# vkit-x/vkit

Measured on AMD Instinct MI355X. Metric: Mpixels/s (2048^2 RGB, geo+photo chain), higher is better.
Workload: dtype u8

## Files before the change

vkit_amd/csrc/nprand.hip:

```cpp
#include "vkx_internal.h"
#include "np_ziggurat.h"

#include <string.h>
#include <algorithm>

namespace {

typedef unsigned __int128 u128;
#define VKX_GLOBAL __attribute__((address_space(1)))

#ifndef VKX_NP_ROUNDS
#define VKX_NP_ROUNDS 48
#endif
constexpr int kRounds = VKX_NP_ROUNDS;
static_assert(kRounds % 2 == 0 && kRounds >= 2 && kRounds <= 64, "rounds per tile");
constexpr int kTile = 64 * kRounds;
constexpr double kNorR = 3.6541528853610087963519472518;
constexpr double kNorInvR = 0.27366123732975827203338247596;

#define PCG_MULT ((((u128)0x2360ED051FC65DA4ull) << 64) | (u128)0x4385DF649FCCF645ull)

struct JumpTabs {
    uint64_t pow2[64][4];
    uint64_t lane[64][4];
    uint64_t a64[2], g64[2];
    uint64_t a128[2], g128[2];
};
static JumpTabs g_jump_host;
static bool g_jump_host_ready = false;

static void jump_consts(u128 j, u128 *a, u128 *g)
{
    u128 acc_mult = 1, acc_plus = 0, cur_mult = PCG_MULT, cur_plus = 1;
    while (j > 0) {
        if (j & 1) {
            acc_mult *= cur_mult;
            acc_plus = acc_plus * cur_mult + cur_plus;
        }
        cur_plus = (cur_mult + 1) * cur_plus;
        cur_mult *= cur_mult;
        j >>= 1;
    }
    *a = acc_mult;
    *g = acc_plus;
}

static void build_jump_tabs()
{
    if (g_jump_host_ready) return;
    auto put = [](uint64_t *w, u128 a, u128 g) {
        w[0] = (uint64_t)a; w[1] = (uint64_t)(a >> 64); w[2] = (uint64_t)g; w[3] = (uint64_t)(g >> 64);
    };
    u128 a, g;
    for (int i = 0; i < 64; i++) { jump_consts((u128)1 << i, &a, &g); put(g_jump_host.pow2[i], a, g); }
    for (int l = 0; l < 64; l++) { jump_consts((u128)(l + 1), &a, &g); put(g_jump_host.lane[l], a, g); }
    jump_consts(64, &a, &g);
    g_jump_host.a64[0] = (uint64_t)a; g_jump_host.a64[1] = (uint64_t)(a >> 64);
    g_jump_host.g64[0] = (uint64_t)g; g_jump_host.g64[1] = (uint64_t)(g >> 64);
    jump_consts(128, &a, &g);
    g_jump_host.a128[0] = (uint64_t)a; g_jump_host.a128[1] = (uint64_t)(a >> 64);
    g_jump_host.g128[0] = (uint64_t)g; g_jump_host.g128[1] = (uint64_t)(g >> 64);
    g_jump_host_ready = true;
}

struct NpTabs {
    JumpTabs jump;
    uint64_t ki[256], wi[256], fi[256];
};

struct NpJob {
    uint64_t state[2], inc[2];
    uint64_t c64[2];
    uint64_t c128[2];
    long long n;
    long long tile_base;
    int n_tiles;
    int kind, cn;
    double loc, scale;
    double margin;
    double cdf[3];
    const uint8_t *src;
    void *dst;
    int16_t *rec;
    uint2 *table;
};

struct TileInfo {
    uint32_t count0, out0;
    uint64_t start0, emit0;
};
constexpr uint32_t kIrregular = 0x80000000u;
struct TilePlan {
    unsigned long long prefix;
    uint32_t c_in, count;
};

__device__ __forceinline__ u128 mk128(const uint64_t *w) { return ((u128)w[1] << 64) | (u128)w[0]; }

__device__ __forceinline__ uint64_t pcg_out(u128 s)
{
    const uint64_t hi = (uint64_t)(s >> 64), lo = (uint64_t)s;
    const uint64_t x = hi ^ lo;
    const unsigned r = (unsigned)(hi >> 58);
    return (x >> r) | (x << ((64 - r) & 63));
}
struct LcgStride {
    uint32_t a0, a1, a2, a3;
    uint64_t c0, c1, c23;
};
__device__ __forceinline__ LcgStride lcg_stride(u128 a, u128 c)
{
    LcgStride k;
    k.a0 = (uint32_t)a; k.a1 = (uint32_t)(a >> 32); k.a2 = (uint32_t)(a >> 64); k.a3 = (uint32_t)(a >> 96);
    k.c0 = (uint32_t)c; k.c1 = (uint32_t)(c >> 32); k.c23 = (uint64_t)(c >> 64);
    return k;
}
__device__ __forceinline__ uint64_t mad_u64_u32_v(uint32_t a, uint32_t b, uint64_t c)
{
    uint64_t d, carry;
    asm("v_mad_u64_u32 %0, %1, %2, %3, %4" : "=v"(d), "=s"(carry) : "v"(a), "v"(b), "v"(c));
    return d;
}
__device__ __forceinline__ uint64_t mul_u64_u32_v(uint32_t a, uint32_t b)
{
    uint64_t d, carry;
    asm("v_mad_u64_u32 %0, %1, %2, %3, 0" : "=v"(d), "=s"(carry) : "v"(a), "v"(b));
    return d;
}
__device__ __forceinline__ u128 lcg_step(u128 s, const LcgStride &k)
{
    const uint32_t s0 = (uint32_t)s, s1 = (uint32_t)(s >> 32), s2 = (uint32_t)(s >> 64), s3 = (uint32_t)(s >> 96);
    const uint64_t E = (uint64_t)k.a0 * s0 + k.c0;
    const uint64_t O1 = (uint64_t)k.a0 * s1 + k.c1;
    const uint64_t O2 = (uint64_t)k.a1 * s0;
    uint64_t F = (uint64_t)k.a0 * s2 + k.c23;
    F += (uint64_t)k.a1 * s1;
    F += (uint64_t)k.a2 * s0;
    uint64_t G = mul_u64_u32_v(k.a0, s3);
    G = mad_u64_u32_v(k.a1, s2, G);
    G = mad_u64_u32_v(k.a2, s1, G);
    G = mad_u64_u32_v(k.a3, s0, G);
    unsigned ca, cb, cc, cd;
    const uint32_t t = __builtin_addc((uint32_t)(E >> 32), (uint32_t)O1, 0u, &ca);
    const uint32_t r1 = __builtin_addc(t, (uint32_t)O2, 0u, &cb);
    const uint32_t u = __builtin_addc((uint32_t)F, (uint32_t)(O1 >> 32), ca, &cc);
    const uint32_t r2 = __builtin_addc(u, (uint32_t)(O2 >> 32), cb, &cd);
    unsigned ce;
    const uint32_t w = __builtin_addc((uint32_t)(F >> 32), (uint32_t)G, cc, &ce);
    const uint32_t r3 = __builtin_addc(w, 0u, cd, &ce);
    return ((u128)r3 << 96) | ((u128)r2 << 64) | ((u128)r1 << 32) | (uint32_t)E;
}

__device__ __forceinline__ double u2dbl(uint64_t u) { return (double)(long long)(u >> 11) * (1.0 / 9007199254740992.0); }

__device__ __forceinline__ int rounded_step(const NpJob &job, double z, bool inexact, uint32_t &flags)
{
    const double v = job.scale * z;
    if (inexact) {
        const double f = v - floor(v);
        if (fabs(f - 0.5) < 1e-9) flags |= VKX_NP_AMBIGUOUS;
    }
    return (int16_t)(int)__double_as_longlong(v + 6755399441055744.0);
}
struct EmitNone {
    typedef int Val;
    typedef int16_t Store;
    __device__ static Val make(const NpJob &, double, bool, uint32_t &) { return 0; }
    __device__ static void store(const NpJob &, void *, long long, Val, bool, uint32_t &) {}
};
struct EmitI16 {
    static constexpr bool kCheckAtStore = false;
    typedef int Val;
    typedef int16_t Store;
    __device__ static Val make(const NpJob &job, double z, bool inexact, uint32_t &flags) { return rounded_step(job, z, inexact, flags); }
    __device__ static void store(const NpJob &, void *dst, long long pos, Val k, bool, uint32_t &) { ((int16_t VKX_GLOBAL *)dst)[pos] = (int16_t)k; }
};
struct EmitAddU8 {
    static constexpr bool kCheckAtStore = false;
    typedef int Val;
    typedef int16_t Store;
    __device__ static Val make(const NpJob &job, double z, bool inexact, uint32_t &flags) { return rounded_step(job, z, inexact, flags); }
    __device__ static void store(const NpJob &job, void *dst, long long pos, Val k, bool, uint32_t &)
    {
        const int s = (int16_t)((int)((const uint8_t VKX_GLOBAL *)job.src)[pos] + k);
        ((uint8_t VKX_GLOBAL *)dst)[pos] = (uint8_t)vkd::clamp_u8(s);
    }
};
struct EmitSpeckle {
    static constexpr bool kCheckAtStore = true;
    typedef double Val;
    typedef double Store;
    __device__ static Val make(const NpJob &, double z, bool, uint32_t &) { return z; }
    __device__ static void store(const NpJob &job, void *dst, long long pos, Val z, bool inexact, uint32_t &flags)
    {
        const double noise = 0.0 + job.scale * z;
        const double m = (double)((const uint8_t VKX_GLOBAL *)job.src)[pos];
        const double t = m * noise;
        double r = m + t;
        if (inexact && m != 0.0 && fabs(r - rint(r)) < 1e-9) flags |= VKX_NP_AMBIGUOUS;
        r = r < 0.0 ? 0.0 : (r > 255.0 ? 255.0 : r);
        ((uint8_t VKX_GLOBAL *)dst)[pos] = (uint8_t)(int)r;
    }
};

constexpr int kEvCap = kRounds <= 48 ? 96 : 128;
template <typename Val, bool WITH_VAL>
struct WaveWork {
    uint64_t ev_s[kEvCap][2];
    uint16_t ev_pos[kEvCap];
    uint16_t ev_info[kEvCap];
    uint64_t slow[kRounds];
    uint64_t semit[kRounds];
    uint64_t cov[kRounds];
    __attribute__((aligned(16))) Val val[WITH_VAL ? kRounds : 1][64];
};

__device__ __forceinline__ uint64_t rfl64(uint64_t v)
{
    return ((uint64_t)(uint32_t)__builtin_amdgcn_readfirstlane((int)(v >> 32)) << 32) | (uint32_t)__builtin_amdgcn_readfirstlane((int)v);
}
__device__ __forceinline__ int mbcnt64(uint64_t m)
{
    return __builtin_amdgcn_mbcnt_hi((uint32_t)(m >> 32), __builtin_amdgcn_mbcnt_lo((uint32_t)m, 0u));
}

enum { kCount = 0, kRecord = 1, kEmit = 2, kCompact = 3 };

__device__ __forceinline__ uint32_t lds_offset(const void *p)
{
    return (uint32_t)(uintptr_t)(__attribute__((address_space(3))) const void *)p;
}

__device__ __forceinline__ uint32_t compact_tile_lds(int16_t *flat, uint64_t m)
{
    const uint32_t lane = (uint32_t)__lane_id();
    const uint32_t base = lds_offset(flat);
    uint32_t run = 0;
    constexpr int kBatch = 8;
    static_assert(kRounds % kBatch == 0 || kRounds < kBatch, "rounds per compaction batch");
#pragma unroll
    for (int r0 = 0; r0 < kRounds; r0 += kBatch) {
        uint32_t v[kBatch];
#pragma unroll
        for (int j = 0; j < kBatch; j++)
            if (r0 + j < kRounds) v[j] = (uint16_t)flat[64 * (r0 + j) + lane];
#pragma unroll
        for (int j = 0; j < kBatch; j++) {
            const int r = r0 + j;
            if (r >= kRounds) break;
            const uint32_t lo = (uint32_t)__builtin_amdgcn_readlane((int)m, r), hi = (uint32_t)__builtin_amdgcn_readlane((int)(m >> 32), r);
            const uint32_t rank = (uint32_t)__builtin_amdgcn_mbcnt_hi(hi, __builtin_amdgcn_mbcnt_lo(lo, run));
            const uint32_t addr = base + 2 * rank;
            const uint64_t mask = ((uint64_t)hi << 32) | lo;
            uint64_t saved;
            asm volatile("s_mov_b64 %[sv], exec\n\ts_mov_b64 exec, %[m]\n\tds_write_b16 %[a], %[v]\n\ts_mov_b64 exec, %[sv]"
                         : [sv] "=&s"(saved) : [m] "s"(mask), [a] "v"(addr), [v] "v"(v[j]) : "memory");
            run += (uint32_t)__builtin_popcountll(mask);
        }
    }
    __builtin_amdgcn_wave_barrier();
    return run;
}

template <class Emit, int MODE>
__device__ void walk_tile(const NpJob &job, const JumpTabs &g_jump, const uint4 *__restrict__ zig , const double *__restrict__ fi ,
                          WaveWork<typename Emit::Store, MODE == kEmit || MODE == kCompact> &ws, u128 base, uint32_t c_in, long long prefix,
                          long long draw_base, typename Emit::Store VKX_GLOBAL *rec_val, uint64_t VKX_GLOBAL *rec_mask, void *emit_dst,
                          uint32_t &count_out, uint32_t &carry_out, uint64_t &start0, uint64_t &emit0, bool &has_tail, uint32_t &flags,
                          unsigned long long *draws_used)
{
    const int lane = __lane_id();
    const u128 inc = mk128(job.inc);
    const u128 a64 = mk128(g_jump.a64), c64 = mk128(job.c64);
    c_in = (uint32_t)__builtin_amdgcn_readfirstlane((int)c_in);
    prefix = (long long)rfl64((uint64_t)prefix);
    draw_base = (long long)rfl64((uint64_t)draw_base);
    u128 s = mk128(&g_jump.lane[lane][0]) * base + mk128(&g_jump.lane[lane][2]) * inc;
    uint32_t nev = 0;
    if (lane < kRounds) ws.semit[lane] = 0;
    auto round = [&](int r, const u128 &st) {
        const uint64_t u = pcg_out(st);
        const int idx = (int)(u & 0xff);
        const uint64_t rabs = (u >> 9) & 0x000fffffffffffffull;
        const uint4 e = zig[idx];
        const uint64_t ki = ((uint64_t)e.y << 32) | e.x;
        if (MODE != kCount) {
            const double wi = __longlong_as_double(((long long)e.w << 32) | e.z);
            double x = (__longlong_as_double((long long)(0x4330000000000000ull | rabs)) - 4503599627370496.0) * wi;
            x = __longlong_as_double(__double_as_longlong(x) | ((long long)((uint32_t)u << 23 & 0x80000000u) << 32));
            const typename Emit::Store v = (typename Emit::Store)Emit::make(job, x, false, flags);
            if (MODE == kRecord) rec_val[64 * r + lane] = v;
            else if (MODE == kEmit || MODE == kCompact) ws.val[r][lane] = v;
        }
        const uint64_t slow = __ballot(rabs >= ki);
        if (lane == 0) ws.slow[r] = slow;
        if (slow) {
            if (rabs >= ki) {
                const uint32_t slot = nev + (uint32_t)mbcnt64(slow);
                if (slot < (uint32_t)kEvCap) {
                    ws.ev_s[slot][0] = (uint64_t)st;
                    ws.ev_s[slot][1] = (uint64_t)(st >> 64);
                    ws.ev_pos[slot] = (uint16_t)(64 * r + lane);
                }
            }
            nev += (uint32_t)__builtin_popcountll(slow);
        }
    };
    const LcgStride stride128 = lcg_stride(mk128(g_jump.a128), mk128(job.c128));
    u128 s2 = a64 * s + c64;
#pragma unroll 1
    for (int r = 0; r < kRounds; r += 2) {
        round(r, s);
        round(r + 1, s2);
        s = lcg_step(s, stride128);
        s2 = lcg_step(s2, stride128);
    }
    if (nev > (uint32_t)kEvCap) {
        flags |= VKX_NP_SHORT;
        nev = kEvCap;
    }
    __builtin_amdgcn_wave_barrier();
    if (MODE == kRecord) asm volatile("s_waitcnt vmcnt(0)" ::: "memory");
    has_tail = false;
#pragma unroll
    for (int q = 0; q < (kEvCap + 63) / 64; q++) {
        if ((uint32_t)(64 * q) >= nev) break;
        const uint32_t ev = 64 * q + lane;
        if (ev < nev) {
            const u128 se = ((u128)ws.ev_s[ev][1] << 64) | ws.ev_s[ev][0];
            const int pos = ws.ev_pos[ev];
            const uint64_t u = pcg_out(se);
            const int idx = (int)(u & 0xff);
            const uint64_t rabs = (u >> 9) & 0x000fffffffffffffull;
            uint32_t info;
            if (idx != 0) {
                double x = (__longlong_as_double((long long)(0x4330000000000000ull | rabs)) - 4503599627370496.0) *
                           __longlong_as_double(((long long)zig[idx].w << 32) | zig[idx].z);
                if (u & 0x100) x = -x;
                const double un = u2dbl(pcg_out(PCG_MULT * se + inc));
                const double f1 = fi[idx], f0 = fi[idx - 1];
                const double lhs = (f0 - f1) * un + f1;
                const double t = -0.5 * x;
                const double y = t * x;
                const float r32 = __builtin_amdgcn_exp2f((float)y * 1.44269504f);
                const float l32 = (float)lhs;
                bool accept = l32 < r32;
                if (fabsf(l32 - r32) <= r32 * 0x1p-14f || job.margin >= 1.0) {
                    const double rhs = exp(y);
                    if (fabs(rhs - lhs) <= lhs * job.margin) flags |= VKX_NP_AMBIGUOUS;
                    accept = lhs < rhs;
                }
                info = 2u | (accept ? 0x100u : 0u);
            } else {
                u128 t = se;
                uint32_t len = 1;
                double xx;
                for (;;) {
                    t = PCG_MULT * t + inc;
                    const double u1 = u2dbl(pcg_out(t));
                    t = PCG_MULT * t + inc;
                    const double u2 = u2dbl(pcg_out(t));
                    len += 2;
                    xx = -kNorInvR * log1p(-u1);
                    const double yy = -log1p(-u2);
                    const double l2 = yy + yy, r2 = xx * xx;
                    if (fabs(l2 - r2) <= r2 * 0x1p-40) flags |= VKX_NP_AMBIGUOUS;
                    if (l2 > r2 || len > 200) break;
                }
                if (len > 200) flags |= VKX_NP_SHORT;
                const double z = ((rabs >> 8) & 1) ? -(kNorR + xx) : kNorR + xx;
                if (MODE == kRecord) {
                    rec_val[pos] = (typename Emit::Store)Emit::make(job, z, true, flags);
                } else if (MODE == kCompact) {
                    (&ws.val[0][0])[pos] = (typename Emit::Store)Emit::make(job, z, true, flags);
                } else if (MODE == kEmit) {
                    const typename Emit::Val v = Emit::make(job, z, true, flags);
                    uint64_t bits = 0;
                    memcpy(&bits, &v, sizeof v);
                    ws.ev_s[ev][0] = bits;
                }
                has_tail = true;
                info = len | 0x300u;
            }
            ws.ev_info[ev] = (uint16_t)info;
            if (info & 0x100u) atomicOr((unsigned long long *)&ws.semit[pos >> 6], 1ull << (pos & 63));
        }
    }
    __builtin_amdgcn_wave_barrier();
    has_tail = __ballot(has_tail) != 0;
    uint32_t P = 0xffffu, end = 0, info = 0;
    if ((uint32_t)lane < nev) {
        P = ws.ev_pos[lane];
        info = ws.ev_info[lane];
        end = P + (info & 0xffu);
    }
    uint64_t valid;
    uint32_t carry = c_in > (uint32_t)kTile ? c_in - kTile : 0u;
    if (nev <= 64) {
        const uint32_t prev_end = (uint32_t)__builtin_amdgcn_update_dpp((int)c_in, (int)end, 0x138 , 0xf, 0xf, false);
        const uint64_t live = nev == 64 ? ~0ull : ((1ull << nev) - 1);
        const uint64_t touch = __ballot((uint32_t)lane < nev && P < prev_end);
        valid = live;
        if (touch) {
            uint32_t cover_end = c_in;
            valid = 0;
            for (uint32_t e = 0; e < nev; e++) {
                const uint32_t pe = (uint32_t)__builtin_amdgcn_readlane((int)P, (int)e);
                if (pe >= cover_end) {
                    valid |= 1ull << e;
                    cover_end = (uint32_t)__builtin_amdgcn_readlane((int)end, (int)e);
                }
            }
        }
        if (valid) {
            const uint32_t last_end = (uint32_t)__builtin_amdgcn_readlane((int)end, 63 - __builtin_clzll(valid));
            if (last_end > (uint32_t)kTile && last_end - kTile > carry) carry = last_end - kTile;
        }
        if (lane < kRounds) ws.cov[lane] = 0;
        __builtin_amdgcn_wave_barrier();
        if ((valid >> lane) & 1) {
            uint32_t p0 = P + 1, p1 = end < (uint32_t)kTile ? end : (uint32_t)kTile;
            while (p0 < p1) {
                const uint32_t r = p0 >> 6, stop = (r + 1) << 6 < p1 ? (r + 1) << 6 : p1;
                const uint32_t lo = p0 & 63, n = stop - p0;
                const uint64_t bits = (n == 64 ? ~0ull : ((1ull << n) - 1)) << lo;
                atomicOr((unsigned long long *)&ws.cov[r], bits);
                p0 = stop;
            }
        }
        __builtin_amdgcn_wave_barrier();
    } else {
        valid = 0;
        if (lane < kRounds) ws.cov[lane] = 0;
        __builtin_amdgcn_wave_barrier();
        uint32_t cover_end = c_in;
        for (uint32_t e = 0; e < nev; e++) {
            const uint32_t pe = ws.ev_pos[e], ee = pe + (ws.ev_info[e] & 0xffu);
            if (pe < cover_end) continue;
            cover_end = ee;
            if (lane == 0)
                for (uint32_t q = pe + 1; q < ee && q < (uint32_t)kTile; q++) ws.cov[q >> 6] |= 1ull << (q & 63);
        }
        if (cover_end > (uint32_t)kTile && cover_end - kTile > carry) carry = cover_end - kTile;
        __builtin_amdgcn_wave_barrier();
    }
    uint64_t my_mask = 0, my_starts = 0;
    if (lane < kRounds) {
        uint64_t cov = ws.cov[lane];
        const uint32_t lo = 64u * lane;
        if (c_in > lo) cov |= c_in - lo >= 64 ? ~0ull : ((1ull << (c_in - lo)) - 1);
        const uint64_t slow = ws.slow[lane];
        my_starts = ~cov;
        my_mask = my_starts & (~slow | ws.semit[lane]);
    }
    start0 = rfl64(my_starts);
    emit0 = rfl64(my_mask);
    uint32_t count = (uint32_t)__builtin_popcountll(my_mask);
    count += (uint32_t)__builtin_amdgcn_update_dpp(0, (int)count, 0x118 , 0xf, 0xf, true);
    count += (uint32_t)__builtin_amdgcn_update_dpp(0, (int)count, 0x114 , 0xf, 0xf, true);
    count += (uint32_t)__builtin_amdgcn_update_dpp(0, (int)count, 0x112 , 0xf, 0xf, true);
    count += (uint32_t)__builtin_amdgcn_update_dpp(0, (int)count, 0x111 , 0xf, 0xf, true);
    {
        uint32_t total = (uint32_t)__builtin_amdgcn_readlane((int)count, 15);
        if (kRounds > 16) total += (uint32_t)__builtin_amdgcn_readlane((int)count, 31);
        if (kRounds > 32) total += (uint32_t)__builtin_amdgcn_readlane((int)count, 47);
        if (kRounds > 48) total += (uint32_t)__builtin_amdgcn_readlane((int)count, 63);
        count = total;
    }
    if (MODE == kEmit) {
        uint32_t done = 0, ebase = 0;
#pragma unroll 1
        for (int r = 0; r < kRounds; r++) {
            if (prefix + done >= job.n) break;
            const uint64_t emits = ((uint64_t)(uint32_t)__builtin_amdgcn_readlane((int)(my_mask >> 32), r) << 32) |
                                   (uint32_t)__builtin_amdgcn_readlane((int)my_mask, r);
            const uint64_t slow = rfl64(ws.slow[r]);
            const bool mine = (emits >> lane) & 1;
            const long long pos = prefix + done + mbcnt64(emits);
            if (mine && pos < job.n) {
                typename Emit::Val z = (typename Emit::Val)ws.val[r][lane];
                bool inexact = false;
                int len = 1;
                if ((slow >> lane) & 1) {
                    const uint32_t ev = ebase + (uint32_t)mbcnt64(slow);
                    const uint32_t einfo = ws.ev_info[ev];
                    len = (int)(einfo & 0xff);
                    if (einfo & 0x200u) {
                        const uint64_t bits = ws.ev_s[ev][0];
                        memcpy(&z, &bits, sizeof z);
                        inexact = true;
                    }
                }
                Emit::store(job, emit_dst, pos, z, inexact, flags);
                if (pos == job.n - 1)
                    __hip_atomic_store(draws_used, (unsigned long long)(draw_base + 64 * r + lane + len), __ATOMIC_RELAXED, __HIP_MEMORY_SCOPE_AGENT);
            }
            done += (uint32_t)__builtin_popcountll(emits);
            ebase += (uint32_t)__builtin_popcountll(slow);
        }
    }
    if (MODE == kRecord && lane < kRounds) rec_mask[lane] = my_mask;
    if constexpr (MODE == kCompact) {
        static_assert(sizeof(typename Emit::Store) == 2, "compact records are int16");
        int16_t *flat = (int16_t *)&ws.val[0][0];
        const uint32_t total = compact_tile_lds(flat, my_mask);
        const uint32_t groups = (total + 7) >> 3;
        typedef uint32_t u32x4 __attribute__((ext_vector_type(4)));
        const u32x4 *f16 = (const u32x4 *)flat;
        u32x4 VKX_GLOBAL *s16 = (u32x4 VKX_GLOBAL *)rec_val;
#pragma unroll
        for (int i = 0; i < kTile / 512; i++) {
            const uint32_t idx = (uint32_t)lane + 64u * i;
            if (idx < groups) s16[idx] = f16[idx];
        }
        __builtin_amdgcn_wave_barrier();
    }
    count_out = count;
    carry_out = carry;
}

__device__ __forceinline__ void load_tables(uint4 *zig, double *fi, const NpTabs *__restrict__ tabs)
{
    for (int i = threadIdx.x; i < 256; i += blockDim.x) {
        const uint64_t k = tabs->ki[i], w = tabs->wi[i];
        zig[i] = make_uint4((uint32_t)k, (uint32_t)(k >> 32), (uint32_t)w, (uint32_t)(w >> 32));
        fi[i] = __longlong_as_double((long long)tabs->fi[i]);
    }
    __syncthreads();
}

__device__ __forceinline__ int job_of_tile(const NpJob *jobs, int n_jobs, long long tile)
{
    int lo = 0, hi = n_jobs - 1;
    while (lo < hi) {
        const int mid = (lo + hi + 1) >> 1;
        if (jobs[mid].tile_base <= tile) lo = mid; else hi = mid - 1;
    }
    return lo;
}

constexpr int kInlineJobs = 8;
struct NpJobPack { NpJob jobs[kInlineJobs]; };

template <bool INLINE>
__global__ void __launch_bounds__(256) k_np_tile_states(const NpJob *__restrict__ jobs_dev, NpJobPack pack, int n_jobs, long long total_tiles,
                                                        uint64_t *__restrict__ states , NpJob *__restrict__ jobs_out,
                                                        vkx_np_result *__restrict__ results, unsigned *__restrict__ done,
                                                        const NpTabs *__restrict__ tabs)
{
    const NpJob *jobs = INLINE ? pack.jobs : jobs_dev;
    if (blockIdx.x == 0) {
        if (INLINE) {
            const uint32_t *src = (const uint32_t *)pack.jobs;
            uint32_t *dst = (uint32_t *)jobs_out;
            for (unsigned i = threadIdx.x; i < (unsigned)n_jobs * (sizeof(NpJob) / 4); i += 256) dst[i] = src[i];
        }
        uint32_t *r = (uint32_t *)results;
        for (unsigned i = threadIdx.x; i < (unsigned)n_jobs * (sizeof(vkx_np_result) / 4); i += 256) r[i] = 0;
        if (threadIdx.x == 0) *done = 0;
    }
    const JumpTabs &g_jump = tabs->jump;
    const long long tile = (long long)blockIdx.x * 256 + threadIdx.x;
    if (tile >= total_tiles) return;
    const NpJob &job = jobs[job_of_tile(jobs, n_jobs, tile)];
    unsigned long long d = (unsigned long long)(tile - job.tile_base) * kTile;
    u128 s = mk128(job.state);
    const u128 inc = mk128(job.inc);
    for (int i = 0; d; i++, d >>= 1)
        if (d & 1) s = mk128(&g_jump.pow2[i][0]) * s + mk128(&g_jump.pow2[i][2]) * inc;
    states[2 * tile] = (uint64_t)s;
    states[2 * tile + 1] = (uint64_t)(s >> 64);
}

__device__ __forceinline__ void np_results_out(unsigned *done, const vkx_np_result *results, vkx_np_result *results_host, int n_jobs)
{
    if (!results_host) return;
    __shared__ bool s_last;
    asm volatile("s_waitcnt vmcnt(0)" ::: "memory");
    __syncthreads();
    if (threadIdx.x == 0) s_last = atomicAdd(done, 1u) == gridDim.x - 1;
    __syncthreads();
    if (!s_last) return;
    const uint32_t *src = (const uint32_t *)results;
    uint32_t *dst = (uint32_t *)results_host;
    for (unsigned i = threadIdx.x; i < (unsigned)n_jobs * (sizeof(vkx_np_result) / 4); i += blockDim.x)
        dst[i] = __hip_atomic_load(src + i, __ATOMIC_RELAXED, __HIP_MEMORY_SCOPE_AGENT);
}

template <class Emit>
__global__ void __launch_bounds__(256) k_np_draw(const NpJob *__restrict__ jobs, int n_jobs, long long total_tiles,
                                                 const uint64_t *__restrict__ states, TileInfo *__restrict__ info,
                                                 typename Emit::Store *__restrict__ rec_val, uint64_t *__restrict__ rec_mask,
                                                 vkx_np_result *__restrict__ results, const NpTabs *__restrict__ tabs)
{
    __shared__ uint4 zig[256];
    __shared__ double fi[256];
    __shared__ WaveWork<typename Emit::Store, false> work[4];
    load_tables(zig, fi, tabs);
    const JumpTabs &g_jump = tabs->jump;
    const long long n_waves = (long long)gridDim.x * 4;
    for (long long tile = (long long)blockIdx.x * 4 + (threadIdx.x >> 6); tile < total_tiles; tile += n_waves) {
        const int j = job_of_tile(jobs, n_jobs, tile);
        const NpJob &job = jobs[j];
        uint32_t count, carry, flags = 0;
        uint64_t start0, emit0;
        bool has_tail;
        walk_tile<Emit, kRecord>(job, g_jump, zig, fi, work[threadIdx.x >> 6], mk128(&states[2 * tile]), 0u, 0, 0,
                                 (typename Emit::Store VKX_GLOBAL *)(rec_val + tile * kTile), (uint64_t VKX_GLOBAL *)(rec_mask + tile * kRounds),
                                 nullptr, count, carry, start0, emit0, has_tail, flags, nullptr);
        if (__lane_id() == 0) {
            TileInfo t;
            t.count0 = count; t.out0 = carry | (has_tail ? 0x80000000u : 0u); t.start0 = start0; t.emit0 = emit0;
            info[tile] = t;
        }
        if (flags) atomicOr(&results[j].flags, flags);
    }
}

constexpr int kSlot = kTile + 16;
#ifndef VKX_NP_DRAW_WAVES
#define VKX_NP_DRAW_WAVES 8
#endif
constexpr int kDrawWaves = VKX_NP_DRAW_WAVES;

template <class Emit>
__global__ void __launch_bounds__(64 * kDrawWaves) k_np_draw_compact(const NpJob *__restrict__ jobs, int n_jobs, long long total_tiles,
                                                                    const uint64_t *__restrict__ states, TileInfo *__restrict__ info,
                                                                    vkx_np_result *__restrict__ results, const NpTabs *__restrict__ tabs)
{
    __shared__ uint4 zig[256];
    __shared__ double fi[256];
    __shared__ WaveWork<int16_t, true> work[kDrawWaves];
    load_tables(zig, fi, tabs);
    const JumpTabs &g_jump = tabs->jump;
    const long long n_waves = (long long)gridDim.x * kDrawWaves;
    for (long long tile = (long long)blockIdx.x * kDrawWaves + (threadIdx.x >> 6); tile < total_tiles; tile += n_waves) {
        const int j = job_of_tile(jobs, n_jobs, tile);
        const NpJob &job = jobs[j];
        uint32_t count, carry, flags = 0;
        uint64_t start0, emit0;
        bool has_tail;
        walk_tile<Emit, kCompact>(job, g_jump, zig, fi, work[threadIdx.x >> 6], mk128(&states[2 * tile]), 0u, 0, 0,
                                  (int16_t VKX_GLOBAL *)(job.rec + (tile - job.tile_base) * kSlot), nullptr, nullptr,
                                  count, carry, start0, emit0, has_tail, flags, nullptr);
        if (__lane_id() == 0) {
            TileInfo t;
            t.count0 = count; t.out0 = carry | (has_tail ? 0x80000000u : 0u); t.start0 = start0; t.emit0 = emit0;
            info[tile] = t;
        }
        if (flags) atomicOr(&results[j].flags, flags);
    }
}

__global__ void __launch_bounds__(1024) k_np_resolve(const NpJob *__restrict__ jobs, const uint64_t *__restrict__ states,
                                                     const TileInfo *__restrict__ info_all, TilePlan *__restrict__ plan_all,
                                                     vkx_np_result *__restrict__ results, const NpTabs *__restrict__ tabs)
{
    __shared__ uint4 zig[256];
    __shared__ double fi[256];
    __shared__ WaveWork<int16_t, false> work[1];
    __shared__ unsigned long long part[1024];
    __shared__ uint32_t n_irregular;
    extern __shared__ uint64_t irregular[];
    const NpJob &job = jobs[blockIdx.x];
    const int T = job.n_tiles;
    const TileInfo *info = info_all + job.tile_base;
    TilePlan *plan = plan_all + job.tile_base;
    const uint64_t *st = states + 2 * job.tile_base;
    const int words = (T + 63) >> 6;
    if (threadIdx.x == 0) n_irregular = 0;
    load_tables(zig, fi, tabs);
    const JumpTabs &g_jump = tabs->jump;
    for (int w = threadIdx.x >> 6; w < words; w += 16) {
        const int j = w * 64 + (threadIdx.x & 63);
        bool bad = false;
        if (j < T) {
            const uint32_t c = j ? (info[j - 1].out0 & 0x7fffffffu) : 0u;
            const TileInfo t = info[j];
            const bool ok = c < 64 && ((t.start0 >> c) & 1);
            TilePlan p;
            p.prefix = 0;
            p.c_in = c;
            p.count = ok ? t.count0 - (uint32_t)__builtin_popcountll(t.emit0 & ((1ull << c) - 1)) : 0u;
            plan[j] = p;
            bad = !ok;
        }
        const uint64_t m = __ballot(bad);
        if ((threadIdx.x & 63) == 0) {
            irregular[w] = m;
            if (m) atomicAdd(&n_irregular, (uint32_t)__builtin_popcountll(m));
        }
    }
    __syncthreads();
    if (n_irregular && threadIdx.x < 64) {
        uint32_t flags = 0;
        for (int w = 0; w < words; w++) {
            for (;;) {
                __threadfence_block();
                const uint64_t m = ((volatile uint64_t *)irregular)[w];
                if (!m) break;
                const int b = __builtin_ctzll(m);
                const int j = w * 64 + b;
                const TileInfo t = info[j];
                const uint32_t c = ((volatile TilePlan *)plan)[j].c_in & ~kIrregular;
                const uint32_t out0 = t.out0 & 0x7fffffffu;
                uint32_t count, out;
                bool simulated = false;
                if (c < 64 && ((t.start0 >> c) & 1)) {
                    count = t.count0 - (uint32_t)__builtin_popcountll(t.emit0 & ((1ull << c) - 1));
                    out = out0;
                } else {
                    uint64_t s0, e0;
                    bool ht;
                    walk_tile<EmitNone, kCount>(job, g_jump, zig, fi, work[0], mk128(&st[2 * j]), c, 0, 0, nullptr, nullptr, nullptr, count, out,
                                                s0, e0, ht, flags, nullptr);
                    simulated = true;
                }
                if (threadIdx.x == 0) {
                    plan[j].count = count;
                    plan[j].c_in = c | (simulated ? kIrregular : 0u);
                    irregular[w] = m & ~(1ull << b);
                    if (j + 1 < T && out != out0) {
                        const TileInfo tn = info[j + 1];
                        const bool ok = out < 64 && ((tn.start0 >> out) & 1);
                        plan[j + 1].c_in = out;
                        plan[j + 1].count = ok ? tn.count0 - (uint32_t)__builtin_popcountll(tn.emit0 & ((1ull << out) - 1)) : 0u;
                        const int wn = (j + 1) >> 6;
                        const uint64_t bit = 1ull << ((j + 1) & 63);
                        irregular[wn] = ok ? (irregular[wn] & ~bit) : (irregular[wn] | bit);
                    }
                }
            }
        }
        if (flags && threadIdx.x == 0) atomicOr(&results[blockIdx.x].flags, flags);
    }
    __threadfence_block();
    __syncthreads();
    const int per = (T + 1023) / 1024;
    const int j0 = threadIdx.x * per, j1 = min(T, j0 + per);
    unsigned long long sum = 0;
    for (int j = j0; j < j1; j++) sum += plan[j].count;
    part[threadIdx.x] = sum;
    __syncthreads();
    for (int d = 1; d < 1024; d <<= 1) {
        const unsigned long long v = threadIdx.x >= d ? part[threadIdx.x - d] : 0ull;
        __syncthreads();
        part[threadIdx.x] += v;
        __syncthreads();
    }
    unsigned long long run = part[threadIdx.x] - sum;
    bool short_tile = false;
    for (int j = j0; j < j1; j++) {
        plan[j].prefix = run;
        short_tile = short_tile || ((long long)run < job.n && j + 1 < T && plan[j].count < 192u);
        run += plan[j].count;
    }
    if (short_tile && job.kind == VKX_NP_NORMAL_TILES) atomicOr(&results[blockIdx.x].flags, VKX_NP_SHORT);
    if (threadIdx.x == 1023) {
        results[blockIdx.x].samples = part[1023];
        if ((long long)part[1023] < job.n) atomicOr(&results[blockIdx.x].flags, VKX_NP_SHORT);
    }
}

template <class Emit>
struct Placer {
    struct Draws {};
    __device__ static Draws load(const typename Emit::Store *) { return Draws(); }
    __device__ static void place(const NpJob &job, const Draws &, const typename Emit::Store *__restrict__ rec, uint64_t m, long long prefix,
                                 typename Emit::Store *, uint32_t &flags)
{
    const typename Emit::Store VKX_GLOBAL *vals = (const typename Emit::Store VKX_GLOBAL *)rec;
    const int lane = __lane_id();
    uint32_t count = 0;
#pragma unroll 4
    for (int r = 0; r < kRounds; r++) {
        const uint64_t emits = ((uint64_t)(uint32_t)__builtin_amdgcn_readlane((int)(m >> 32), r) << 32) |
                               (uint32_t)__builtin_amdgcn_readlane((int)m, r);
        const long long pos = prefix + count + mbcnt64(emits);
        if (((emits >> lane) & 1) && pos < job.n) Emit::store(job, job.dst, pos, (typename Emit::Val)vals[64 * r + lane], false, flags);
        count += (uint32_t)__builtin_popcountll(emits);
    }
}
};

struct TileDraws { uint32_t v[kRounds / 2]; };
__device__ __forceinline__ TileDraws load_tile_i16(const int16_t *__restrict__ rec)
{
    const uint32_t VKX_GLOBAL *vals = (const uint32_t VKX_GLOBAL *)rec;
    const int lane = __lane_id();
    TileDraws d;
#pragma unroll
    for (int q = 0; q < kRounds / 2; q++) d.v[q] = vals[64 * q + lane];
    return d;
}
constexpr int kRawOff = 8;
__device__ __forceinline__ uint32_t stage_tile_lds(const TileDraws &d, uint64_t m, uint32_t shift, int16_t *st)
{
    const uint32_t lane = (uint32_t)__lane_id();
    uint32_t *raw32 = (uint32_t *)(st + kRawOff);
#pragma unroll
    for (int q = 0; q < kRounds / 2; q++) raw32[64 * q + lane] = d.v[q];
    __builtin_amdgcn_wave_barrier();
    const int16_t *raw = st + kRawOff;
    const uint32_t st_addr = lds_offset(st);
    uint32_t run = shift;
#pragma unroll
    for (int r = 0; r < kRounds; r++) {
        const uint32_t lo = (uint32_t)__builtin_amdgcn_readlane((int)m, r), hi = (uint32_t)__builtin_amdgcn_readlane((int)(m >> 32), r);
        const uint32_t rank = (uint32_t)__builtin_amdgcn_mbcnt_hi(hi, __builtin_amdgcn_mbcnt_lo(lo, run));
        const uint32_t v = (uint16_t)raw[64 * r + lane];
        const uint32_t addr = st_addr + 2 * rank;
        const uint64_t mask = ((uint64_t)hi << 32) | lo;
        uint64_t saved;
        asm volatile("s_mov_b64 %[sv], exec\n\ts_mov_b64 exec, %[m]\n\tds_write_b16 %[a], %[v]\n\ts_mov_b64 exec, %[sv]"
                     : [sv] "=&s"(saved) : [m] "s"(mask), [a] "v"(addr), [v] "v"(v) : "memory");
        run += (uint32_t)__builtin_popcountll(mask);
    }
    __builtin_amdgcn_wave_barrier();
    return run - shift;
}


template <>
struct Placer<EmitI16> {
    typedef TileDraws Draws;
    __device__ static Draws load(const int16_t *rec) { return load_tile_i16(rec); }
    __device__ static void place(const NpJob &job, const Draws &d, const int16_t *, uint64_t m, long long prefix, int16_t *st, uint32_t &)
{
    const uint32_t shift = (uint32_t)prefix & 1u;
    uint32_t total = stage_tile_lds(d, m, shift, st);
    if (prefix + total > job.n) total = (uint32_t)(job.n - prefix);
    finish(job, total, shift, prefix, st);
}
    __device__ static void finish(const NpJob &job, uint32_t total, uint32_t shift, long long prefix, int16_t *st)
{
    const uint32_t lane = (uint32_t)__lane_id();
    int16_t VKX_GLOBAL *dst = (int16_t VKX_GLOBAL *)job.dst + (prefix - shift);
    const uint32_t end = shift + total;
    const uint32_t full_hi = end >> 1;
    uint32_t VKX_GLOBAL *dst32 = (uint32_t VKX_GLOBAL *)dst + lane;
    const uint32_t *st32 = (const uint32_t *)st + lane;
    if (lane >= shift && lane < full_hi) dst32[0] = st32[0];
#pragma unroll
    for (uint32_t i = 1; i < kTile / 128; i++)
        if (lane + 64 * i < full_hi) dst32[64 * i] = st32[64 * i];
    if (lane == 0) {
        if (shift && end > 1) dst[1] = st[1];
        if ((end & 1) && end - 1 >= shift) dst[end - 1] = st[end - 1];
    }
    __builtin_amdgcn_wave_barrier();
}
};

template <>
struct Placer<EmitAddU8> {
    typedef TileDraws Draws;
    __device__ static Draws load(const int16_t *rec) { return load_tile_i16(rec); }
    __device__ static void place(const NpJob &job, const Draws &d, const int16_t *, uint64_t m, long long prefix, int16_t *st, uint32_t &)
{
    const uint32_t shift = (uint32_t)prefix & 3u;
    const uint32_t lane = (uint32_t)__lane_id();
    const long long first = prefix - shift;
    const uint32_t VKX_GLOBAL *src32 = (const uint32_t VKX_GLOBAL *)((const uint8_t VKX_GLOBAL *)job.src + first) + lane;
    uint32_t px[kTile / 256];
#pragma unroll
    for (uint32_t i = 0; i < kTile / 256; i++) {
        px[i] = 0;
        if (first + 4 * (long long)(lane + 64 * i) + 3 < job.n) px[i] = src32[64 * i];
    }
    uint32_t total = stage_tile_lds(d, m, shift, st);
    if (prefix + total > job.n) total = (uint32_t)(job.n - prefix);
    finish_px(job, total, shift, prefix, st, px);
}
    __device__ static void finish(const NpJob &job, uint32_t total, uint32_t shift, long long prefix, int16_t *st)
{
    const uint32_t lane = (uint32_t)__lane_id();
    const long long first = prefix - shift;
    const uint32_t VKX_GLOBAL *src32 = (const uint32_t VKX_GLOBAL *)((const uint8_t VKX_GLOBAL *)job.src + first) + lane;
    uint32_t px[kTile / 256];
#pragma unroll
    for (uint32_t i = 0; i < kTile / 256; i++) {
        px[i] = 0;
        if (first + 4 * (long long)(lane + 64 * i) + 3 < job.n) px[i] = src32[64 * i];
    }
    finish_px(job, total, shift, prefix, st, px);
}
    __device__ static void finish_px(const NpJob &job, uint32_t total, uint32_t shift, long long prefix, int16_t *st,
                                     const uint32_t (&pxs)[kTile / 256])
{
    typedef short pk16 __attribute__((ext_vector_type(2)));
    const uint32_t lane = (uint32_t)__lane_id();
    const uint8_t VKX_GLOBAL *src = (const uint8_t VKX_GLOBAL *)job.src + (prefix - shift);
    uint8_t VKX_GLOBAL *dst = (uint8_t VKX_GLOBAL *)job.dst + (prefix - shift);
    const uint32_t end = shift + total;
    const uint32_t full_lo = (shift + 3) >> 2, full_hi = end >> 2;
    uint32_t VKX_GLOBAL *dst32 = (uint32_t VKX_GLOBAL *)dst + lane;
    const uint2 *st64 = (const uint2 *)st + lane;
    auto whole = [&](uint32_t i) {
        const uint32_t px = pxs[i];
        const uint2 nz = st64[64 * i];
        pk16 lo = __builtin_bit_cast(pk16, __builtin_amdgcn_perm(0u, px, 0x0c010c00u));
        pk16 hi = __builtin_bit_cast(pk16, __builtin_amdgcn_perm(0u, px, 0x0c030c02u));
        lo += __builtin_bit_cast(pk16, nz.x);
        hi += __builtin_bit_cast(pk16, nz.y);
        const pk16 zero = {0, 0}, top = {255, 255};
        lo = __builtin_elementwise_min(__builtin_elementwise_max(lo, zero), top);
        hi = __builtin_elementwise_min(__builtin_elementwise_max(hi, zero), top);
        dst32[64 * i] = __builtin_amdgcn_perm(__builtin_bit_cast(uint32_t, hi), __builtin_bit_cast(uint32_t, lo), 0x06040200u);
    };
    if (lane >= full_lo && lane < full_hi) whole(0);
#pragma unroll
    for (uint32_t i = 1; i < kTile / 256; i++)
        if (lane + 64 * i < full_hi) whole(i);
    if (lane < 8) {
        const uint32_t e = lane < 4 ? lane : 4 * full_hi + (lane - 4);
        const bool mine = lane < 4 ? (shift > 0 && e >= shift && e < end) : (e < end && !(full_hi == 0 && shift > 0));
        if (mine) dst[e] = (uint8_t)vkd::clamp_u8((int16_t)((int)src[e] + (int)st[e]));
    }
    __builtin_amdgcn_wave_barrier();
}
};

__device__ __forceinline__ bool tile_needs_walk(const NpJob &job, const TilePlan &p, uint32_t out0, bool check_at_store)
{
    return (p.c_in & kIrregular) || (long long)p.prefix + p.count >= job.n || (check_at_store && (out0 >> 31));
}

template <class Emit>
__global__ void __launch_bounds__(256) k_np_place(const NpJob *__restrict__ jobs, int n_jobs, long long total_tiles,
                                                  const TileInfo *__restrict__ info, const TilePlan *__restrict__ plan,
                                                  const typename Emit::Store *__restrict__ rec_val, const uint64_t *__restrict__ rec_mask,
                                                  vkx_np_result *__restrict__ results)
{
    __shared__ __attribute__((aligned(16))) typename Emit::Store stage[4][kTile + 64];
    const int lane = __lane_id();
// ... 644 lines not shown
```

Before: 64900.

## Pack draw pairs into 32-bit LDS words and restructure ziggurat round pipeline

Reworks the ziggurat draw loop so it computes the table lookup for two PCG states first and finishes them afterwards. Mantissa and exponent assembly now uses alignbit and bitop3, and the exponent bias is folded into the ki table so the slow-path comparison works on the built double bits. In compact mode, pairs of int16 values are written as one packed 32-bit LDS word and read back as pairs, using ds_write_b16_d16_hi for odd rounds. The slow-path index writes are remapped with park_index to match this layout, and the per-round slow ballot store is replaced by atomics in the slow path. The aim is fewer ALU ops and LDS transactions per draw, at the cost of more complex indexing and a higher risk of layout bugs.

After: 66690 (median of 6 runs). +2.8%, better.

```diff
diff --git a/vkit_amd/csrc/nprand.hip b/vkit_amd/csrc/nprand.hip
--- a/vkit_amd/csrc/nprand.hip
+++ b/vkit_amd/csrc/nprand.hip
@@ -95,6 +95,7 @@
     uint32_t c_in, count;
 };
 
+typedef uint32_t u32x4 __attribute__((ext_vector_type(4)));
 __device__ __forceinline__ u128 mk128(const uint64_t *w) { return ((u128)w[1] << 64) | (u128)w[0]; }
 
 __device__ __forceinline__ uint64_t pcg_out(u128 s)
@@ -160,7 +161,7 @@
         const double f = v - floor(v);
         if (fabs(f - 0.5) < 1e-9) flags |= VKX_NP_AMBIGUOUS;
     }
-    return (int16_t)(int)__double_as_longlong(v + 6755399441055744.0);
+    return (int)(uint32_t)__double_as_longlong(v + 6755399441055744.0);
 }
 struct EmitNone {
     typedef int Val;
@@ -231,19 +232,22 @@
     return (uint32_t)(uintptr_t)(__attribute__((address_space(3))) const void *)p;
 }
 
+__device__ __forceinline__ uint32_t park_index(uint32_t pos) { return (pos & ~127u) | ((pos & 63u) << 1) | ((pos >> 6) & 1u); }
+
 __device__ __forceinline__ uint32_t compact_tile_lds(int16_t *flat, uint64_t m)
 {
     const uint32_t lane = (uint32_t)__lane_id();
     const uint32_t base = lds_offset(flat);
+    const uint32_t *pairs = (const uint32_t *)flat;
     uint32_t run = 0;
     constexpr int kBatch = 8;
     static_assert(kRounds % kBatch == 0 || kRounds < kBatch, "rounds per compaction batch");
 #pragma unroll
     for (int r0 = 0; r0 < kRounds; r0 += kBatch) {
-        uint32_t v[kBatch];
+        uint32_t v[kBatch / 2];
 #pragma unroll
-        for (int j = 0; j < kBatch; j++)
-            if (r0 + j < kRounds) v[j] = (uint16_t)flat[64 * (r0 + j) + lane];
+        for (int j = 0; j < kBatch; j += 2)
+            if (r0 + j < kRounds) v[j / 2] = pairs[32 * (r0 + j) + lane];
 #pragma unroll
         for (int j = 0; j < kBatch; j++) {
             const int r = r0 + j;
@@ -253,8 +257,12 @@
             const uint32_t addr = base + 2 * rank;
             const uint64_t mask = ((uint64_t)hi << 32) | lo;
             uint64_t saved;
-            asm volatile("s_mov_b64 %[sv], exec\n\ts_mov_b64 exec, %[m]\n\tds_write_b16 %[a], %[v]\n\ts_mov_b64 exec, %[sv]"
-                         : [sv] "=&s"(saved) : [m] "s"(mask), [a] "v"(addr), [v] "v"(v[j]) : "memory");
+            if (j & 1)
+                asm volatile("s_mov_b64 %[sv], exec\n\ts_mov_b64 exec, %[m]\n\tds_write_b16_d16_hi %[a], %[v]\n\ts_mov_b64 exec, %[sv]"
+                             : [sv] "=&s"(saved) : [m] "s"(mask), [a] "v"(addr), [v] "v"(v[j / 2]) : "memory");
+            else
+                asm volatile("s_mov_b64 %[sv], exec\n\ts_mov_b64 exec, %[m]\n\tds_write_b16 %[a], %[v]\n\ts_mov_b64 exec, %[sv]"
+                             : [sv] "=&s"(saved) : [m] "s"(mask), [a] "v"(addr), [v] "v"(v[j / 2]) : "memory");
             run += (uint32_t)__builtin_popcountll(mask);
         }
     }
@@ -277,25 +285,39 @@
     draw_base = (long long)rfl64((uint64_t)draw_base);
     u128 s = mk128(&g_jump.lane[lane][0]) * base + mk128(&g_jump.lane[lane][2]) * inc;
     uint32_t nev = 0;
-    if (lane < kRounds) ws.semit[lane] = 0;
-    auto round = [&](int r, const u128 &st) {
+    if (lane < kRounds) {
+        ws.semit[lane] = 0;
+        ws.slow[lane] = 0;
+    }
+    struct Draw {
+        uint32_t lo, dlo, dhi;
+        u32x4 e;
+    };
+    uint32_t k_m20 = 0x000fffffu, k_exp = 0x43300000u, k_sgn = 0x80000000u;
+    asm volatile("" : "+v"(k_m20), "+v"(k_exp), "+v"(k_sgn));
+    auto lookup = [&](const u128 &st) {
         const uint64_t u = pcg_out(st);
-        const int idx = (int)(u & 0xff);
-        const uint64_t rabs = (u >> 9) & 0x000fffffffffffffull;
-        const uint4 e = zig[idx];
-        const uint64_t ki = ((uint64_t)e.y << 32) | e.x;
+        Draw d;
+        d.lo = (uint32_t)u;
+        d.e = ((const u32x4 *)zig)[d.lo & 0xff];
+        d.dlo = __builtin_amdgcn_alignbit((uint32_t)(u >> 32), d.lo, 9);
+        d.dhi = __builtin_amdgcn_bitop3_b32((uint32_t)(u >> 41), k_m20, k_exp, 0xea );
+        return d;
+    };
+    auto finish = [&](int r, const u128 &st, const Draw &d) -> typename Emit::Val {
+        typename Emit::Val v = 0;
         if (MODE != kCount) {
-            const double wi = __longlong_as_double(((long long)e.w << 32) | e.z);
-            double x = (__longlong_as_double((long long)(0x4330000000000000ull | rabs)) - 4503599627370496.0) * wi;
-            x = __longlong_as_double(__double_as_longlong(x) | ((long long)((uint32_t)u << 23 & 0x80000000u) << 32));
-            const typename Emit::Store v = (typename Emit::Store)Emit::make(job, x, false, flags);
-            if (MODE == kRecord) rec_val[64 * r + lane] = v;
-            else if (MODE == kEmit || MODE == kCompact) ws.val[r][lane] = v;
-        }
-        const uint64_t slow = __ballot(rabs >= ki);
-        if (lane == 0) ws.slow[r] = slow;
+            const uint32_t wsgn = __builtin_amdgcn_bitop3_b32(__builtin_amdgcn_alignbit(d.lo, d.lo, 9), k_sgn, d.e[3], 0xea);
+            const double wi = __longlong_as_double(((long long)wsgn << 32) | d.e[2]);
+            const double x = (__longlong_as_double((long long)(((uint64_t)d.dhi << 32) | d.dlo)) - 4503599627370496.0) * wi;
+            v = Emit::make(job, x, false, flags);
+            if (MODE == kRecord) rec_val[64 * r + lane] = (typename Emit::Store)v;
+            else if (MODE == kEmit) ws.val[r][lane] = (typename Emit::Store)v;
+        }
+        const bool slow_me = (((uint64_t)d.dhi << 32) | d.dlo) >= (((uint64_t)d.e[1] << 32) | d.e[0]);
+        const uint64_t slow = __ballot(slow_me);
         if (slow) {
-            if (rabs >= ki) {
+            if (slow_me) {
                 const uint32_t slot = nev + (uint32_t)mbcnt64(slow);
                 if (slot < (uint32_t)kEvCap) {
                     ws.ev_s[slot][0] = (uint64_t)st;
@@ -305,15 +327,20 @@
             }
             nev += (uint32_t)__builtin_popcountll(slow);
         }
+        return v;
     };
     const LcgStride stride128 = lcg_stride(mk128(g_jump.a128), mk128(job.c128));
     u128 s2 = a64 * s + c64;
-#pragma unroll 1
+#pragma unroll 2
     for (int r = 0; r < kRounds; r += 2) {
-        round(r, s);
-        round(r + 1, s2);
+        const u128 sa = s, sb = s2;
+        const Draw da = lookup(sa), db = lookup(sb);
         s = lcg_step(s, stride128);
         s2 = lcg_step(s2, stride128);
+        const typename Emit::Val va = finish(r, sa, da);
+        const typename Emit::Val vb = finish(r + 1, sb, db);
+        if constexpr (MODE == kCompact)
+            ((uint32_t *)&ws.val[0][0])[32 * r + lane] = __builtin_amdgcn_perm((uint32_t)vb, (uint32_t)va, 0x05040100u);
     }
     if (nev > (uint32_t)kEvCap) {
         flags |= VKX_NP_SHORT;
@@ -372,7 +399,7 @@
                 if (MODE == kRecord) {
                     rec_val[pos] = (typename Emit::Store)Emit::make(job, z, true, flags);
                 } else if (MODE == kCompact) {
-                    (&ws.val[0][0])[pos] = (typename Emit::Store)Emit::make(job, z, true, flags);
+                    (&ws.val[0][0])[park_index(pos)] = (typename Emit::Store)Emit::make(job, z, true, flags);
                 } else if (MODE == kEmit) {
                     const typename Emit::Val v = Emit::make(job, z, true, flags);
                     uint64_t bits = 0;
@@ -383,6 +410,7 @@
                 info = len | 0x300u;
             }
             ws.ev_info[ev] = (uint16_t)info;
+            atomicOr((unsigned long long *)&ws.slow[pos >> 6], 1ull << (pos & 63));
             if (info & 0x100u) atomicOr((unsigned long long *)&ws.semit[pos >> 6], 1ull << (pos & 63));
         }
     }
@@ -505,7 +533,6 @@
         int16_t *flat = (int16_t *)&ws.val[0][0];
         const uint32_t total = compact_tile_lds(flat, my_mask);
         const uint32_t groups = (total + 7) >> 3;
-        typedef uint32_t u32x4 __attribute__((ext_vector_type(4)));
         const u32x4 *f16 = (const u32x4 *)flat;
         u32x4 VKX_GLOBAL *s16 = (u32x4 VKX_GLOBAL *)rec_val;
 #pragma unroll
@@ -523,7 +550,7 @@
 {
     for (int i = threadIdx.x; i < 256; i += blockDim.x) {
         const uint64_t k = tabs->ki[i], w = tabs->wi[i];
-        zig[i] = make_uint4((uint32_t)k, (uint32_t)(k >> 32), (uint32_t)w, (uint32_t)(w >> 32));
+        zig[i] = make_uint4((uint32_t)k, (uint32_t)(k >> 32) | 0x43300000u, (uint32_t)w, (uint32_t)(w >> 32));
         fi[i] = __longlong_as_double((long long)tabs->fi[i]);
     }
     __syncthreads();
@@ -628,9 +655,15 @@
                                                                     const uint64_t *__restrict__ states, TileInfo *__restrict__ info,
                                                                     vkx_np_result *__restrict__ results, const NpTabs *__restrict__ tabs)
 {
-    __shared__ uint4 zig[256];
-    __shared__ double fi[256];
-    __shared__ WaveWork<int16_t, true> work[kDrawWaves];
+    struct Lds {
+        uint4 zig[256];
+        double fi[256];
+        WaveWork<int16_t, true> work[kDrawWaves];
+    };
+    __shared__ Lds lds;
+    uint4 *zig = lds.zig;
+    double *fi = lds.fi;
+    WaveWork<int16_t, true> *work = lds.work;
     load_tables(zig, fi, tabs);
     const JumpTabs &g_jump = tabs->jump;
     const long long n_waves = (long long)gridDim.x * kDrawWaves;
```
